# NVIDIA/OpenSeq2Seq

Hardware: AMD Instinct MI355X
Metric: audio-frames/sec/node Jasper10x5 bf16 (train step, objects = input feature frames) (higher is better)
Workload: dtype bf16; 1 GPU; Jasper 10x5 DR (jasper10x5_LibriSpeech_nvgrad_masks) full train step: log-mel front end from int16 PCM resident in HBM+fwd+bwd+NovoGrad/LARC/Backoff, B=32/GPU, durations U[2,16.7]s padded to the batch max, F=64, V=29; global_batch=32, parallelism=dp1, skipped_steps=0

## Files before the change

openseq2seq_amd/csrc/conv1d_wgrad.hip:

```cpp
#include <stdlib.h>

#include <cstdlib>
#include "os2s_common.hpp"
#include "os2s_split_reduce.hpp"
#include <mutex>

namespace os2s {

struct WgradArgs {
  const bf16_t* x;
  const bf16_t* dy;
  float* dw;
  const int32_t* in_len;
  int B, Tin, Tout, Cin, Cout, K, stride, dil, padL;
  int NCO, NCI, NTP, NSPLIT, steps_per_split, use_atomic;
  float* part;
  int xrows, xrows_pad;
  int xbuf_bytes, steptab_bytes;
  long long x_ld;
  int accumulate;
  float* ws_slabs;
  int* ws_cnt;
  int ws_nslabs, ncu, force_split;
  int xcd_order;
  int NG;
  const bf16_t* gx[8];
  const bf16_t* gdy[8];
  float* gdw[8];
  unsigned long long* dbg;
  int dbg_mode;
};

__device__ __forceinline__ int wgrad_xcd_rank(int b, int n) {
  const int q = n >> 3, r = n & 7, x = b & 7;
  return (x < r ? x * (q + 1) : r * (q + 1) + (x - r) * q) + (b >> 3);
}

__device__ __forceinline__ void dma16w(const void* gsrc, char* lds_wave_base) {
  __builtin_amdgcn_global_load_lds(
      (const __attribute__((address_space(1))) void*)gsrc,
      (__attribute__((address_space(3))) void*)lds_wave_base, 16, 0, 0);
}

__device__ __forceinline__ bf16x4 lds_tr(const char* p) {
  return __builtin_amdgcn_ds_read_tr16_b64_v4bf16(
      (__attribute__((address_space(3))) bf16x4*)p);
}

template <int TAPS, int COT>
__device__ __forceinline__ void wgrad_lockstep_unit(const WgradArgs& p, const int unit, const int tp, char* smem) {
  constexpr int BT = 64;
  constexpr int NW = COT / 32, NTHR = NW * 64, NSUB = COT / 128;
  const int tid = threadIdx.x, lane = tid & 63;
  const int wid = __builtin_amdgcn_readfirstlane(tid >> 6);
  const int wm = wid >> 1, wn = wid & 1;
  const int ysub = wm >> 1, wmi = wm & 1;
  const int split = unit / (p.NCO * p.NCI);
  const int rem = unit - split * (p.NCO * p.NCI);
  const int co0 = (rem / p.NCI) * COT, ci0 = (rem % p.NCI) * 128;
  const int k0 = tp * TAPS;
  const int ntaps = min(TAPS, p.K - k0);

  const int ybuf_bytes = NSUB * BT * 256;
  const int xbuf_bytes = p.xrows_pad * 256;
  char* const ybuf0 = smem;
  char* const xbuf0 = smem + 2 * ybuf_bytes;
  const char* const zero = reinterpret_cast<const char*>(g_zero_page);

  const int tchunks = (p.Tout + BT - 1) / BT;
  auto nlive = [&](int b) -> int {
    if (!p.in_len) return tchunks;
    const int l = min(max(p.in_len[b], 0), p.Tin);
    if (l <= 0) return 0;
    return min(tchunks, (l + p.padL + BT * p.stride - 1) / (BT * p.stride));
  };
  int total_live = 0;
  for (int b = 0; b < p.B; ++b) total_live += nlive(b);
  const int sps = (total_live + p.NSPLIT - 1) / p.NSPLIT;
  const int s_begin = split * sps;
  const int s_end = min(total_live, s_begin + sps);
  const int nsteps = max(0, s_end - s_begin);
  int cur_b = 0, cur_c = 0;
  {
    int acc_steps = 0;
    while (cur_b < p.B && acc_steps + nlive(cur_b) <= s_begin) { acc_steps += nlive(cur_b); ++cur_b; }
    cur_c = s_begin - acc_steps;
  }

  auto stage = [&](int step, int buf) {
    const int b = min(cur_b, p.B - 1);
    const int t0 = cur_c * BT;
    ++cur_c;
    if (cur_c >= nlive(b)) {
      cur_c = 0;
      ++cur_b;
      while (cur_b < p.B && nlive(cur_b) == 0) ++cur_b;
    }
    int len_b = p.Tin;
    if (p.in_len) {
      int l = p.in_len[b];
      len_b = l < 0 ? 0 : (l < p.Tin ? l : p.Tin);
    }
    char* yd = ybuf0 + buf * ybuf_bytes;
    const bf16_t* dyb = p.dy + (long long)b * p.Tout * p.Cout;
#pragma unroll
    for (int it = 0; it < (NSUB * 16) / NW; ++it) {
      const int base = (it * NW + wid) * 64;
      const int q = base + lane;
      const int sub = q >> 10, row = (q & 1023) >> 4, ps = q & 15;
      const int u = (ps >> 1) ^ ((row & 3) << 1);
      const int ch = co0 + sub * 128 + ((u << 1) | (ps & 1)) * 8;
      const int t = t0 + row;
      const bool ok = (t < p.Tout) && (ch < p.Cout);
      const void* src = ok ? (const void*)(dyb + (long long)t * p.Cout + ch)
                           : (const void*)(zero + ps * 16);
      dma16w(src, yd + base * 16);
    }
    char* xd = xbuf0 + buf * xbuf_bytes;
    const bf16_t* xb = p.x + (long long)b * p.Tin * p.x_ld;
    const int tin0 = t0 * p.stride + k0 * p.dil - p.padL;
    const int npieces = p.xrows_pad * 16;
    for (int base = wid * 64; base < npieces; base += NTHR) {
      const int q = base + lane;
      const int row = q >> 4, ps = q & 15;
      const int u = (ps >> 1) ^ ((row & 3) << 1);
      const int ch = ci0 + ((u << 1) | (ps & 1)) * 8;
      const int tin = tin0 + row;
      const bool ok = (row < p.xrows) && (tin >= 0) && (tin < len_b) && (ch < p.Cin);
      const void* src = ok ? (const void*)(xb + (long long)tin * p.x_ld + ch)
                           : (const void*)(zero + ps * 16);
      dma16w(src, xd + base * 16);
    }
  };

  f32x16 acc[TAPS][2][2];
#pragma unroll
  for (int a = 0; a < TAPS; ++a)
#pragma unroll
    for (int i = 0; i < 2; ++i)
#pragma unroll
      for (int j = 0; j < 2; ++j)
#pragma unroll
        for (int e = 0; e < 16; ++e) acc[a][i][j][e] = 0.f;

  const int g16 = (lane >> 4) & 1;
  const int i16 = lane & 15;
  const int rsub = i16 >> 2;
  const int csub = (i16 & 3) * 8;
  const int lhi = lane >> 5;

  if (nsteps > 0) stage(0, 0);
  for (int step = 0; step < nsteps; ++step) {
    asm volatile("s_waitcnt vmcnt(0)" ::: "memory");
    __syncthreads();
    if (step + 1 < nsteps) stage(step + 1, (step + 1) & 1);
    const char* const ys = ybuf0 + (step & 1) * ybuf_bytes + ysub * (BT * 256);
    const char* const xs = xbuf0 + (step & 1) * xbuf_bytes;
    struct Frags { bf16x8 af[2]; bf16x8 bfr[TAPS][2]; };
    auto load_frags = [&](int kk) {
      Frags f;
#pragma unroll
      for (int i = 0; i < 2; ++i) {
        const int u = ((wmi * 64 + i * 32) >> 4) + g16;
        const int r0 = kk * 16 + lhi * 8 + rsub;
        const int r1 = r0 + 4;
        const bf16x4 lo = lds_tr(ys + r0 * 256 + ((u ^ ((r0 & 3) << 1)) << 5) + csub);
        const bf16x4 hi = lds_tr(ys + r1 * 256 + ((u ^ ((r1 & 3) << 1)) << 5) + csub);
        f.af[i] = __builtin_shufflevector(lo, hi, 0, 1, 2, 3, 4, 5, 6, 7);
      }
#pragma unroll
      for (int a = 0; a < TAPS; ++a)
#pragma unroll
        for (int j = 0; j < 2; ++j) {
          const int u = ((wn * 64 + j * 32) >> 4) + g16;
          const int r0 = (kk * 16 + lhi * 8 + rsub) * p.stride + a * p.dil;
          const int r1 = r0 + 4 * p.stride;
// ... 562 lines not shown
      const int row = qq >> 4, ps = qq & 15;
      const int u = (ps >> 1) ^ ((row & 3) << 1);
      const int ch = ci0 + (idx >> 4) * 128 + ((u << 1) | (ps & 1)) * 8;
      xv[it] = ch < p.Cin ? (row * (int)p.x_ld + ch) * 2 : (int)0x80000000;
    }
  }
  const unsigned long long dy_base = (unsigned long long)p.dy, x_base = (unsigned long long)p.x;
  const int ycol_bytes = __builtin_amdgcn_readfirstlane(p.Cout * 2);
  const int xcol_bytes = __builtin_amdgcn_readfirstlane((int)p.x_ld * 2);
  auto entry = [&](int i, int& b, int& t0, int& len_b) {
    const unsigned long long m = __ballot(scan <= i);
    int bb = __builtin_popcountll(m);
    bb = bb < p.B ? bb : p.B - 1;
    b = __builtin_amdgcn_readfirstlane(bb);
    const int before = b > 0 ? __builtin_amdgcn_readlane(scan, b - 1) : 0;
    t0 = (i - before) * BT;
    len_b = __builtin_amdgcn_readlane(len_l, b);
  };
  auto stage_y = [&](int b, int t0, int len_b, int slot) {
    int rows = len_b - t0;
    rows = rows < 0 ? 0 : (rows > BT ? BT : rows);
    rows = __builtin_amdgcn_readfirstlane(rows);
    const unsigned long long base =
        dy_base + ((unsigned long long)(unsigned)b * (unsigned)p.Tout + (unsigned)t0) * (unsigned)ycol_bytes;
    const __amdgpu_buffer_rsrc_t rs = __builtin_amdgcn_make_buffer_rsrc((void*)base, 0, rows * ycol_bytes, 0x00020000);
    char* const dst = smem + slot * TILE + grp * HALF;
#pragma unroll
    for (int it = 0; it < 4; ++it)
      __builtin_amdgcn_raw_ptr_buffer_load_lds(
          rs, (__attribute__((address_space(3))) void*)(dst + (it * 4 + wn) * 1024), 16, yv[it], 0, 0, 0);
  };
  auto stage_x = [&](int b, int t0, int len_b, int slot) {
    int rows = len_b - t0;
    rows = rows < 0 ? 0 : (rows > BT ? BT : rows);
    rows = __builtin_amdgcn_readfirstlane(rows);
    const unsigned long long base =
        x_base + ((unsigned long long)(unsigned)b * (unsigned)p.Tin + (unsigned)t0) * (unsigned)xcol_bytes;
    const __amdgpu_buffer_rsrc_t rs = __builtin_amdgcn_make_buffer_rsrc((void*)base, 0, rows * xcol_bytes, 0x00020000);
    char* const dst = smem + 3 * TILE + slot * TILE;
#pragma unroll
    for (int it = 0; it < 4; ++it)
      __builtin_amdgcn_raw_ptr_buffer_load_lds(
          rs, (__attribute__((address_space(3))) void*)(dst + (it * 8 + wid) * 1024), 16, xv[it], 0, 0, 0);
  };

  f32x16 acc[2][2][2];
#pragma unroll
  for (int e = 0; e < 2; ++e)
#pragma unroll
    for (int i = 0; i < 2; ++i)
#pragma unroll
      for (int j = 0; j < 2; ++j)
#pragma unroll
        for (int v = 0; v < 16; ++v) acc[e][i][j][v] = 0.f;

  const int lhi = lane >> 5;
  if (nsteps > 0) {
    const int g16 = (lane >> 4) & 1, i16 = lane & 15;
    const int rsub = i16 >> 2, csub = (i16 & 3) * 8;
    int ya[2][2], xa[2];
#pragma unroll
    for (int e = 0; e < 2; ++e)
#pragma unroll
      for (int i = 0; i < 2; ++i) {
        const int u = 4 * e + 2 * i + g16;
        ya[e][i] = grp * HALF + (lhi * 8 + rsub) * 256 + ((u ^ ((rsub & 3) << 1)) << 5) + csub;
      }
#pragma unroll
    for (int j = 0; j < 2; ++j) {
      const int u = 4 * (wn & 1) + 2 * j + g16;
      xa[j] = (wn >> 1) * HALF + (lhi * 8 + rsub) * 256 + ((u ^ ((rsub & 3) << 1)) << 5) + csub;
    }
    {
      int b, t0, len_b;
      entry(s_begin, b, t0, len_b);
      stage_y(b, t0, len_b, 0);
      stage_x(b, t0, len_b, 0);
      if (nsteps > 1) {
        entry(s_begin + 1, b, t0, len_b);
        stage_y(b, t0, len_b, 1);
        stage_x(b, t0, len_b, 1);
        asm volatile("s_waitcnt vmcnt(8)" ::: "memory");
      } else {
        asm volatile("s_waitcnt vmcnt(0)" ::: "memory");
      }
    }
    wpp_barrier();
    if (grp) wpp_barrier();

    const unsigned lds0 = (unsigned)(size_t)(__attribute__((address_space(3))) void*)smem;
    int yi = 0;
    for (int s = 0; s < nsteps; ++s) {
      const unsigned ys = lds0 + yi * TILE;
      const unsigned xs = lds0 + 3 * TILE + (s & 1) * TILE;
      const bool more = s + 2 < nsteps;
      bf16x8 xf[2][4], yf[2][4];
#pragma unroll
      for (int j = 0; j < 2; ++j) {
        xf[j][0] = lds_frag<0>(xs + xa[j]); xf[j][1] = lds_frag<1>(xs + xa[j]);
        xf[j][2] = lds_frag<2>(xs + xa[j]); xf[j][3] = lds_frag<3>(xs + xa[j]);
      }
#pragma unroll
      for (int i = 0; i < 2; ++i) {
        yf[i][0] = lds_frag<0>(ys + ya[0][i]); yf[i][1] = lds_frag<1>(ys + ya[0][i]);
        yf[i][2] = lds_frag<2>(ys + ya[0][i]); yf[i][3] = lds_frag<3>(ys + ya[0][i]);
      }
      int b2 = 0, t2 = 0, l2 = 0;
      if (more) {
        entry(s_begin + s + 2, b2, t2, l2);
        int y2 = yi + 2;
        y2 = y2 >= 3 ? y2 - 3 : y2;
        stage_y(b2, t2, l2, y2);
      }
      asm volatile("s_waitcnt lgkmcnt(0)" ::: "memory");
      wpp_barrier();
#pragma unroll
      for (int kk = 0; kk < 4; ++kk)
#pragma unroll
        for (int i = 0; i < 2; ++i)
#pragma unroll
          for (int j = 0; j < 2; ++j)
            acc[0][i][j] = __builtin_amdgcn_mfma_f32_32x32x16_bf16(yf[i][kk], xf[j][kk], acc[0][i][j], 0, 0, 0);
      wpp_barrier();
#pragma unroll
      for (int i = 0; i < 2; ++i) {
        yf[i][0] = lds_frag<0>(ys + ya[1][i]); yf[i][1] = lds_frag<1>(ys + ya[1][i]);
        yf[i][2] = lds_frag<2>(ys + ya[1][i]); yf[i][3] = lds_frag<3>(ys + ya[1][i]);
      }
      if (more) {
        asm volatile("s_waitcnt vmcnt(4)" ::: "memory");
        stage_x(b2, t2, l2, s & 1);
      } else {
        asm volatile("s_waitcnt vmcnt(0)" ::: "memory");
      }
      yi = yi + 1 >= 3 ? 0 : yi + 1;
      asm volatile("s_waitcnt lgkmcnt(0)" ::: "memory");
      wpp_barrier();
#pragma unroll
      for (int kk = 0; kk < 4; ++kk)
#pragma unroll
        for (int i = 0; i < 2; ++i)
#pragma unroll
          for (int j = 0; j < 2; ++j)
            acc[1][i][j] = __builtin_amdgcn_mfma_f32_32x32x16_bf16(yf[i][kk], xf[j][kk], acc[1][i][j], 0, 0, 0);
      wpp_barrier();
    }
    if (!grp) wpp_barrier();
  }
  __syncthreads();

  if (npiece > 1) {
    const int sidx = rank - nfull;
    auto at = [&](int v) -> f32x16& { return acc[v >> 2][(v >> 1) & 1][v & 1]; };
    if (!split_publish_and_reduce(at, p.ws_slabs + (size_t)sidx * f * kSplitSlabFloats,
                                  p.ws_cnt + sidx, piece, f, smem, tid))
      return;
  }

  const int l31 = lane & 31;
  const bool inside = __builtin_amdgcn_readfirstlane((co0 + 256 <= p.Cout && ci0 + 256 <= p.Cin) ? 1 : 0);
#pragma unroll
  for (int e = 0; e < 2; ++e) {
    const int cob = co0 + grp * 128 + e * 64, cib = ci0 + wn * 64;
    if (inside) {
      float* const base = p.dw + (long long)(cob + 4 * lhi) * p.Cin + cib + l31;
      float old[2][2][16];
      if (p.accumulate) {
#pragma unroll
        for (int i = 0; i < 2; ++i)
#pragma unroll
          for (int j = 0; j < 2; ++j)
#pragma unroll
            for (int v = 0; v < 16; ++v)
              old[i][j][v] = base[(long long)(i * 32 + (v & 3) + 8 * (v >> 2)) * p.Cin + j * 32];
#pragma unroll
        for (int i = 0; i < 2; ++i)
#pragma unroll
          for (int j = 0; j < 2; ++j)
#pragma unroll
            for (int v = 0; v < 16; ++v) acc[e][i][j][v] += old[i][j][v];
      }
#pragma unroll
      for (int i = 0; i < 2; ++i)
#pragma unroll
        for (int j = 0; j < 2; ++j)
#pragma unroll
          for (int v = 0; v < 16; ++v)
            base[(long long)(i * 32 + (v & 3) + 8 * (v >> 2)) * p.Cin + j * 32] = acc[e][i][j][v];
    } else {
#pragma unroll
      for (int i = 0; i < 2; ++i)
#pragma unroll
        for (int j = 0; j < 2; ++j) {
          const int ci = cib + j * 32 + l31;
#pragma unroll
          for (int v = 0; v < 16; ++v) {
            const int co = cob + i * 32 + (v & 3) + 8 * (v >> 2) + 4 * lhi;
            if (co < p.Cout && ci < p.Cin) {
              float* dst = p.dw + (long long)co * p.Cin + ci;
              float val = acc[e][i][j][v];
              if (p.accumulate) val += *dst;
              *dst = val;
            }
          }
        }
    }
  }
}

}

static int conv1d_wgrad_impl(os2s_stream_t stream, const uint16_t* x, long long x_row_stride,
                             const uint16_t* dy, float* dw, const int32_t* in_len, int B,
                             int Tin, int Cin, int Cout, int K, int stride, int dil,
                             int padL, int Tout, int accumulate, void* workspace,
                             size_t workspace_bytes);

static int wgrad_pp_min_units() {
  static const int v = [] { const char* e = getenv("OS2S_WGRAD_PP_MIN_UNITS"); return e ? atoi(e) : 8; }();
  return v;
}
static bool wgrad1x1_pp_auto(int B, int T, int Cin, int Cout, bool have_ws) {
  static const int mode = [] { const char* e = getenv("OS2S_WGRAD1X1_PP"); return e ? atoi(e) : -1; }();
  if (mode == 0) return false;
  if (mode == 1) return true;
  const long long rows = (long long)B * T;
  const int units = os2s::ceil_div(Cout, 256) * os2s::ceil_div(Cin, 256);
  return have_ws && rows >= 2048 && units >= 32;
}
static int g_wgrad_variant = -1;
static int g_wgrad_split = -1;
static int g_wgrad_sw_ablate = 0;
static int g_wgrad_xcd = 1;
static unsigned long long* g_wgrad_dbg = nullptr;
static int g_wgrad_dbg_mode = 0;
static os2s::OptionReg r_wg_variant("conv1d_wgrad.variant", [](double v) { g_wgrad_variant = (int)v; });
static os2s::OptionReg r_wg_split("conv1d_wgrad.split", [](double v) { g_wgrad_split = (int)v; });
static os2s::OptionReg r_wg_abl("conv1d_wgrad.sw_ablate", [](double v) { g_wgrad_sw_ablate = (int)v; });
static os2s::OptionReg r_wg_xcd("conv1d_wgrad.xcd_order", [](double v) { g_wgrad_xcd = v != 0 ? 1 : 0; });
static os2s::StampReg r_wg_stamps("conv1d_wgrad", [](void* stamps, int mode) {
  g_wgrad_dbg = (unsigned long long*)stamps;
  g_wgrad_dbg_mode = mode;
});

extern "C" int os2s_conv1d_wgrad_ws(os2s_stream_t stream, const uint16_t* x, long long x_row_stride,
                                    const uint16_t* dy, float* dw, const int32_t* in_len, int B,
                                    int Tin, int Cin, int Cout, int K, int stride, int dil,
                                    int padL, int Tout, int accumulate, void* workspace,
                                    size_t workspace_bytes) {
  return conv1d_wgrad_impl(stream, x, x_row_stride, dy, dw, in_len, B, Tin, Cin, Cout, K, stride,
                           dil, padL, Tout, accumulate, workspace, workspace_bytes);
}

extern "C" int os2s_conv1d_wgrad_ex(os2s_stream_t stream, const uint16_t* x, long long x_row_stride,
                                    const uint16_t* dy, float* dw, const int32_t* in_len, int B,
                                    int Tin, int Cin, int Cout, int K, int stride, int dil,
                                    int padL, int Tout, int accumulate) {
  return conv1d_wgrad_impl(stream, x, x_row_stride, dy, dw, in_len, B, Tin, Cin, Cout, K, stride,
                           dil, padL, Tout, accumulate, nullptr, 0);
}

extern "C" int os2s_conv1d_wgrad(os2s_stream_t stream, const uint16_t* x,
                                 const uint16_t* dy, float* dw,
                                 const int32_t* in_len, int B, int Tin, int Cin,
                                 int Cout, int K, int stride, int dil, int padL,
                                 int Tout, int accumulate) {
  return conv1d_wgrad_impl(stream, x, Cin, dy, dw, in_len, B, Tin, Cin, Cout, K, stride, dil,
                           padL, Tout, accumulate, nullptr, 0);
}

static int conv1d_wgrad_impl_g(os2s_stream_t stream, const uint16_t* x, long long x_row_stride,
                               const uint16_t* dy, float* dw, const int32_t* in_len, int B,
                               int Tin, int Cin, int Cout, int K, int stride, int dil,
                               int padL, int Tout, int accumulate, void* workspace,
                               size_t workspace_bytes, const os2s_cwgrad_group_t* groups, int ngroups);

static int conv1d_wgrad_impl(os2s_stream_t stream, const uint16_t* x, long long x_row_stride,
                             const uint16_t* dy, float* dw, const int32_t* in_len, int B,
                             int Tin, int Cin, int Cout, int K, int stride, int dil,
                             int padL, int Tout, int accumulate, void* workspace,
                             size_t workspace_bytes) {
  return conv1d_wgrad_impl_g(stream, x, x_row_stride, dy, dw, in_len, B, Tin, Cin, Cout, K, stride, dil, padL, Tout,
                             accumulate, workspace, workspace_bytes, nullptr, 1);
}

extern "C" int os2s_conv1d_wgrad_grouped_ws(os2s_stream_t stream, const os2s_cwgrad_group_t* groups, int ngroups,
                                            const int32_t* in_len, int B, int Tin, int Cin, int Cout, int K,
                                            int stride, int dil, int padL, int Tout, int accumulate,
                                            void* workspace, size_t workspace_bytes) {
  OS2S_REQUIRE(groups && ngroups >= 1 && ngroups <= 8);
  for (int i = 0; i < ngroups; ++i) OS2S_REQUIRE(groups[i].x && groups[i].dy && groups[i].dw);
  for (int i = 1; i < ngroups; ++i) OS2S_REQUIRE(groups[i].x_row_stride == groups[0].x_row_stride);
  int rc = OS2S_ERR_UNSUPPORTED;
  if (ngroups > 1)
    rc = conv1d_wgrad_impl_g(stream, groups[0].x, groups[0].x_row_stride, groups[0].dy, groups[0].dw, in_len, B, Tin,
                             Cin, Cout, K, stride, dil, padL, Tout, accumulate, workspace, workspace_bytes, groups,
                             ngroups);
  if (rc != OS2S_ERR_UNSUPPORTED) return rc;
  for (int i = 0; i < ngroups; ++i) {
    rc = conv1d_wgrad_impl(stream, groups[i].x, groups[i].x_row_stride, groups[i].dy, groups[i].dw, in_len, B, Tin,
                           Cin, Cout, K, stride, dil, padL, Tout, accumulate, workspace, workspace_bytes);
    if (rc != OS2S_OK) return rc;
  }
  return OS2S_OK;
}

static int conv1d_wgrad_impl_g(os2s_stream_t stream, const uint16_t* x, long long x_row_stride,
                               const uint16_t* dy, float* dw, const int32_t* in_len, int B,
                               int Tin, int Cin, int Cout, int K, int stride, int dil,
                               int padL, int Tout, int accumulate, void* workspace,
                               size_t workspace_bytes, const os2s_cwgrad_group_t* groups, int ngroups) {
  using namespace os2s;
  OS2S_REQUIRE(x_row_stride >= Cin && x_row_stride % 8 == 0);
  OS2S_REQUIRE(x && dy && dw);
  OS2S_REQUIRE(B >= 0 && Tin >= 1 && Tout >= 1 && Cin >= 8 && Cout >= 8 && K >= 1);
  OS2S_REQUIRE(Cin % 8 == 0 && Cout % 8 == 0 && stride >= 1 && dil >= 1);
  if (B == 0) return OS2S_OK;
  WgradArgs a;
  a.x = x; a.dy = dy; a.dw = dw; a.in_len = in_len;
  a.B = B; a.Tin = Tin; a.Tout = Tout; a.Cin = Cin; a.Cout = Cout; a.K = K;
  a.stride = stride; a.dil = dil; a.padL = padL; a.x_ld = x_row_stride;
  a.accumulate = accumulate ? 1 : 0;
  a.part = nullptr; a.ws_slabs = nullptr; a.ws_cnt = nullptr; a.ws_nslabs = 0; a.ncu = 256; a.force_split = g_wgrad_split;
  a.dbg = g_wgrad_dbg; a.dbg_mode = g_wgrad_dbg_mode; a.xcd_order = g_wgrad_xcd; a.NG = 1;
  for (int i = 0; i < 8; ++i) { a.gx[i] = nullptr; a.gdy[i] = nullptr; a.gdw[i] = nullptr; }
  if (groups) {
    a.NG = ngroups;
    for (int i = 0; i < ngroups; ++i) { a.gx[i] = groups[i].x; a.gdy[i] = groups[i].dy; a.gdw[i] = groups[i].dw; }
  }

  const bool pp_shape = stride == 1 && K >= 2 && B <= 64 && Cout >= 128 && Cin >= 64 &&
                        Tin < 65536 && Tout <= 255 * 64 && 63 + 3 * dil + 1 <= 96 &&
                        (long long)Tin * x_row_stride * 2 < (1ll << 30) &&
                        (long long)Tin * x_row_stride * 2 < (1ll << 31) &&
                        (long long)Tout * Cout * 2 < (1ll << 31);
  const int pp_units = ceil_div(Cout, 128) * ceil_div(Cin, 128) * ceil_div(K, kWppTaps);
  const bool sw_shape = pp_shape && 63 + 3 * dil + 1 <= kSwXInstr * 16 &&
                        Cout % 128 == 0 && Cin % 128 == 0;
  if (sw_shape && g_wgrad_variant == 3 && !groups) {
    a.NCO = ceil_div(Cout, 128);
    a.NCI = ceil_div(Cin, 128);
    a.NTP = ceil_div(K, kWppTaps);
    a.NSPLIT = 1; a.steps_per_split = 0; a.use_atomic = 0;
    a.xrows = 63 + (kWppTaps - 1) * dil + 1;
    a.xrows_pad = ceil_div(a.xrows, 4) * 4;
    a.xbuf_bytes = kSwXBuf;
    a.steptab_bytes = ceil_div(B * ceil_div(Tout, 64) * 4, 16) * 16;
    const size_t smem = (size_t)kSwRing * (kSwYBuf + kSwXBuf) + a.steptab_bytes;
    if (smem <= 160 * 1024) {
      static std::once_flag once_sw;
      static hipError_t attr_rc = hipSuccess;
      static int ncu = 256;
      std::call_once(once_sw, [] {
        attr_rc = hipFuncSetAttribute((const void*)conv1d_wgrad_sw_kernel<0>,
                                      hipFuncAttributeMaxDynamicSharedMemorySize, 160 * 1024);
#ifdef OS2S_SW_ABLATE
        for (const void* k : {(const void*)conv1d_wgrad_sw_kernel<1>, (const void*)conv1d_wgrad_sw_kernel<2>,
                              (const void*)conv1d_wgrad_sw_kernel<4>, (const void*)conv1d_wgrad_sw_kernel<8>,
                              (const void*)conv1d_wgrad_sw_kernel<3>, (const void*)conv1d_wgrad_sw_kernel<5>})
          if (attr_rc == hipSuccess) attr_rc = hipFuncSetAttribute(k, hipFuncAttributeMaxDynamicSharedMemorySize, 160 * 1024);
#endif
        int dev = 0, n = 0;
        if (hipGetDevice(&dev) == hipSuccess &&
            hipDeviceGetAttribute(&n, hipDeviceAttributeMultiprocessorCount, dev) == hipSuccess && n > 0)
          ncu = n;
      });
      if (attr_rc != hipSuccess) return OS2S_ERR_LAUNCH;
      a.ncu = ncu;
      const size_t slab_bytes = (size_t)kSplitSlabFloats * 4;
      if (workspace && workspace_bytes >= kSplitTicketBytes + 2 * slab_bytes) {
        a.ws_cnt = reinterpret_cast<int*>(workspace);
        a.ws_slabs = reinterpret_cast<float*>(reinterpret_cast<char*>(workspace) + kSplitTicketBytes);
        size_t n = (workspace_bytes - kSplitTicketBytes) / slab_bytes;
        const size_t cap = (size_t)3 * ncu;
        a.ws_nslabs = (int)(n < cap ? n : cap);
      }
      const int U = a.NCO * a.NCI * a.NTP;
      const int r = U % ncu;
      const int pieces = a.ws_nslabs < 16 * r ? a.ws_nslabs : 16 * r;
#ifdef OS2S_SW_ABLATE
      switch (g_wgrad_sw_ablate) {
        case 1: OS2S_LAUNCH(conv1d_wgrad_sw_kernel<1>, dim3(U + pieces), dim3(256), smem, (hipStream_t)stream, a); return OS2S_OK;
        case 2: OS2S_LAUNCH(conv1d_wgrad_sw_kernel<2>, dim3(U + pieces), dim3(256), smem, (hipStream_t)stream, a); return OS2S_OK;
        case 3: OS2S_LAUNCH(conv1d_wgrad_sw_kernel<3>, dim3(U + pieces), dim3(256), smem, (hipStream_t)stream, a); return OS2S_OK;
        case 4: OS2S_LAUNCH(conv1d_wgrad_sw_kernel<4>, dim3(U + pieces), dim3(256), smem, (hipStream_t)stream, a); return OS2S_OK;
        case 5: OS2S_LAUNCH(conv1d_wgrad_sw_kernel<5>, dim3(U + pieces), dim3(256), smem, (hipStream_t)stream, a); return OS2S_OK;
        case 8: OS2S_LAUNCH(conv1d_wgrad_sw_kernel<8>, dim3(U + pieces), dim3(256), smem, (hipStream_t)stream, a); return OS2S_OK;
        default: break;
      }
#endif
      OS2S_LAUNCH(conv1d_wgrad_sw_kernel<0>, dim3(U + pieces), dim3(256), smem, (hipStream_t)stream, a);
      return OS2S_OK;
    }
  }

  if (pp_shape && g_wgrad_variant != 0 && (groups || g_wgrad_variant == 1 || pp_units >= wgrad_pp_min_units())) {
    a.NCO = ceil_div(Cout, 128);
    a.NCI = ceil_div(Cin, 128);
    a.NTP = ceil_div(K, kWppTaps);
    a.NSPLIT = 1; a.steps_per_split = 0; a.use_atomic = 0;
    a.xrows = 63 + (kWppTaps - 1) * dil + 1;
    a.xrows_pad = ceil_div(a.xrows, 4) * 4;
    a.xbuf_bytes = 24 * 1024;
    a.steptab_bytes = ceil_div(B * ceil_div(Tout, 64) * 4, 16) * 16;
    const size_t smem = (size_t)2 * 64 * 256 + (size_t)3 * a.xbuf_bytes + a.steptab_bytes + (a.dbg ? 2 * 48 * 10 * 8 : 0);
    if (smem <= 160 * 1024) {
      static std::once_flag once;
      static hipError_t attr_rc = hipSuccess;
      static int ncu = 256;
      std::call_once(once, [] {
        attr_rc = hipFuncSetAttribute((const void*)conv1d_wgrad_pp_kernel<false>,
                                      hipFuncAttributeMaxDynamicSharedMemorySize, 160 * 1024);
        if (attr_rc == hipSuccess)
          attr_rc = hipFuncSetAttribute((const void*)conv1d_wgrad_pp_kernel<true>,
                                        hipFuncAttributeMaxDynamicSharedMemorySize, 160 * 1024);
        int dev = 0, n = 0;
        if (hipGetDevice(&dev) == hipSuccess &&
            hipDeviceGetAttribute(&n, hipDeviceAttributeMultiprocessorCount, dev) == hipSuccess && n > 0)
          ncu = n;
      });
      if (attr_rc != hipSuccess) return OS2S_ERR_LAUNCH;
      a.ncu = ncu;
      const size_t slab_bytes = (size_t)kSplitSlabFloats * 4;
      if (workspace && workspace_bytes >= kSplitTicketBytes + 2 * slab_bytes) {
        a.ws_cnt = reinterpret_cast<int*>(workspace);
        a.ws_slabs = reinterpret_cast<float*>(reinterpret_cast<char*>(workspace) + kSplitTicketBytes);
        size_t n = (workspace_bytes - kSplitTicketBytes) / slab_bytes;
        const size_t cap = (size_t)3 * ncu;
        a.ws_nslabs = (int)(n < cap ? n : cap);
      }
      const int U = a.NG * a.NCO * a.NCI * a.NTP;
      const int r = U % ncu;
      int pieces = a.ws_nslabs < 16 * r ? a.ws_nslabs : 16 * r;
      const int grid = U + pieces;
      if (a.dbg) {
        OS2S_LAUNCH(conv1d_wgrad_pp_kernel<true>, dim3(grid), dim3(512), smem, (hipStream_t)stream, a);
      } else {
        OS2S_LAUNCH(conv1d_wgrad_pp_kernel<false>, dim3(grid), dim3(512), smem, (hipStream_t)stream, a);
      }
      return OS2S_OK;
    }
  }

  if (groups) return OS2S_ERR_UNSUPPORTED;

  const bool pp1_shape = K == 1 && stride == 1 && padL == 0 && Tin == Tout && B <= 64 &&
                         Cout >= 128 && Cin >= 128 && x_row_stride * 2 * 64 < (1ll << 30) &&
                         (long long)Cout * 2 * 64 < (1ll << 30);
  if (pp1_shape && g_wgrad_variant != 0 && g_wgrad_variant != 1 &&
      (g_wgrad_variant == 2 || wgrad1x1_pp_auto(B, Tout, Cin, Cout, workspace != nullptr))) {
    a.NCO = ceil_div(Cout, 256);
    a.NCI = ceil_div(Cin, 256);
    a.NTP = 1;
    a.NSPLIT = 1; a.steps_per_split = 0; a.use_atomic = 0;
    a.xrows = 64; a.xrows_pad = 64; a.xbuf_bytes = 0; a.steptab_bytes = 0;
    static std::once_flag once1;
    static hipError_t attr_rc1 = hipSuccess;
    static int ncu1 = 256;
    std::call_once(once1, [] {
      attr_rc1 = hipFuncSetAttribute((const void*)conv1d_wgrad1x1_pp_kernel,
                                     hipFuncAttributeMaxDynamicSharedMemorySize, 160 * 1024);
      int dev = 0, n = 0;
      if (hipGetDevice(&dev) == hipSuccess &&
          hipDeviceGetAttribute(&n, hipDeviceAttributeMultiprocessorCount, dev) == hipSuccess && n > 0)
        ncu1 = n;
    });
    if (attr_rc1 != hipSuccess) return OS2S_ERR_LAUNCH;
    a.ncu = ncu1;
    const size_t slab_bytes = (size_t)kSplitSlabFloats * 4;
    if (workspace && workspace_bytes >= kSplitTicketBytes + 2 * slab_bytes) {
      a.ws_cnt = reinterpret_cast<int*>(workspace);
      a.ws_slabs = reinterpret_cast<float*>(reinterpret_cast<char*>(workspace) + kSplitTicketBytes);
      size_t n = (workspace_bytes - kSplitTicketBytes) / slab_bytes;
      const size_t cap = (size_t)3 * ncu1;
      a.ws_nslabs = (int)(n < cap ? n : cap);
    }
    const int U = a.NCO * a.NCI;
    const int r = U % ncu1;
    const int pieces = a.ws_nslabs < 16 * r ? a.ws_nslabs : 16 * r;
    WgradGroupTable none;
    none.ngroups = 0; none.total_units = 0;
    OS2S_LAUNCH(conv1d_wgrad1x1_pp_kernel, dim3(U + pieces), dim3(512), (size_t)160 * 1024,
                (hipStream_t)stream, a, none);
    return OS2S_OK;
  }

  const int TAPS = K == 1 ? 1 : 2;
  const bool wide = (Cout % 256 == 0) && (K >= 8) && (Cout >= 512);
  const int COT = wide ? 256 : 128;
  a.NCO = ceil_div(Cout, COT);
  a.NCI = ceil_div(Cin, 128);
  a.NTP = ceil_div(K, TAPS);
  const int base_blocks = a.NCO * a.NCI * a.NTP;
  const int total_steps = B * ceil_div(Tout, 64);
  int nsplit = 1;
  if (accumulate) {
    const int target = wide ? 256 : 512;
    nsplit = ceil_div(target, base_blocks);
    const int max_split = total_steps / 8 > 0 ? total_steps / 8 : 1;
    if (nsplit > max_split) nsplit = max_split;
    if (nsplit < 1) nsplit = 1;
    if (os2s_deterministic()) nsplit = 1;
  }
  const long long dw_elems = (long long)K * Cout * Cin;
  if (workspace) {
    const long long part_room = workspace_bytes > kSplitTicketBytes
                                    ? (long long)((workspace_bytes - kSplitTicketBytes) / ((size_t)dw_elems * 4)) : 0;
    if (nsplit > part_room) nsplit = (int)part_room;
    if (nsplit < 1) nsplit = 1;
  }
  a.steps_per_split = ceil_div(total_steps, nsplit);
  a.NSPLIT = ceil_div(total_steps, a.steps_per_split);
  if (workspace && a.NSPLIT > 1)
    a.part = reinterpret_cast<float*>(reinterpret_cast<char*>(workspace) + kSplitTicketBytes);
  a.use_atomic = (accumulate && !a.part) ? 1 : 0;
  a.xrows = 63 * stride + (TAPS - 1) * dil + 1;
  a.xrows_pad = ceil_div(a.xrows, 4) * 4;
  const size_t smem = (size_t)2 * 64 * 2 * COT + (size_t)2 * a.xrows_pad * 256;
  if (smem > 160 * 1024) return OS2S_ERR_UNSUPPORTED;
  static std::once_flag once2;
  static hipError_t attr_rc2 = hipSuccess;
  std::call_once(once2, [] {
    if (hipFuncSetAttribute((const void*)conv1d_wgrad_kernel<2, 128>,
                            hipFuncAttributeMaxDynamicSharedMemorySize, 160 * 1024) != hipSuccess ||
        hipFuncSetAttribute((const void*)conv1d_wgrad_kernel<2, 256>,
                            hipFuncAttributeMaxDynamicSharedMemorySize, 160 * 1024) != hipSuccess ||
        hipFuncSetAttribute((const void*)conv1d_wgrad_kernel<1, 128>,
                            hipFuncAttributeMaxDynamicSharedMemorySize, 160 * 1024) != hipSuccess ||
        hipFuncSetAttribute((const void*)conv1d_wgrad_kernel<1, 256>,
                            hipFuncAttributeMaxDynamicSharedMemorySize, 160 * 1024) != hipSuccess)
      attr_rc2 = hipErrorUnknown;
  });
  if (attr_rc2 != hipSuccess) return OS2S_ERR_LAUNCH;
  const int nunits = a.NCO * a.NCI * a.NSPLIT;
  const int grid = ceil_div(nunits, 8) * 8 * a.NTP;
  if (wide) {
    if (TAPS == 1)
      OS2S_LAUNCH((conv1d_wgrad_kernel<1, 256>), dim3(grid), dim3(512), smem, (hipStream_t)stream, a);
    else
      OS2S_LAUNCH((conv1d_wgrad_kernel<2, 256>), dim3(grid), dim3(512), smem, (hipStream_t)stream, a);
  } else {
    if (TAPS == 1)
      OS2S_LAUNCH((conv1d_wgrad_kernel<1, 128>), dim3(grid), dim3(256), smem, (hipStream_t)stream, a);
    else
      OS2S_LAUNCH((conv1d_wgrad_kernel<2, 128>), dim3(grid), dim3(256), smem, (hipStream_t)stream, a);
  }
  if (a.part) {
    const int blocks = ceil_div(dw_elems, 256) < 2048 ? ceil_div(dw_elems, 256) : 2048;
    OS2S_LAUNCH(wgrad_split_sum_kernel, dim3(blocks), dim3(256), 0, (hipStream_t)stream,
                (const float*)a.part, dw, dw_elems, a.NSPLIT);
  }
  return OS2S_OK;
}


extern "C" int os2s_conv1x1_wgrad_grouped(os2s_stream_t stream, const os2s_wgrad_group_t* groups, int ngroups,
                                          const int32_t* in_len, int B, int T) {
  using namespace os2s;
  OS2S_REQUIRE(groups && ngroups >= 1 && ngroups <= kMaxWgradGroups && B >= 0 && T >= 1);
  if (B == 0) return OS2S_OK;
  WgradGroupTable gt;
  gt.ngroups = ngroups;
  int tiles = 0;
  for (int i = 0; i < ngroups; ++i) {
    const os2s_wgrad_group_t& s = groups[i];
    OS2S_REQUIRE(s.x && s.dy && s.dw && s.Cin >= 8 && s.Cout >= 8 && s.Cin % 8 == 0 && s.Cout % 8 == 0);
    OS2S_REQUIRE(s.x_row_stride >= s.Cin && s.x_row_stride % 8 == 0);
    tiles += ceil_div(s.Cout, 128) * ceil_div(s.Cin, 128);
  }
  const int total_steps = B * ceil_div(T, 64);
  int nsplit = ceil_div(512, tiles);
  const int max_split = total_steps / 8 > 0 ? total_steps / 8 : 1;
  if (nsplit > max_split) nsplit = max_split;
  if (tiles >= 256 || nsplit < 1 || os2s_deterministic()) nsplit = 1;
  WgradArgs a;
  a.x = nullptr; a.dy = nullptr; a.dw = nullptr; a.in_len = in_len;
  a.B = B; a.Tin = T; a.Tout = T; a.Cin = 0; a.Cout = 0; a.K = 1;
  a.stride = 1; a.dil = 1; a.padL = 0; a.x_ld = 0; a.accumulate = 1;
  a.part = nullptr; a.ws_slabs = nullptr; a.ws_cnt = nullptr; a.ws_nslabs = 0; a.ncu = 256; a.force_split = -1;
  a.dbg = nullptr; a.dbg_mode = 0; a.xcd_order = g_wgrad_xcd; a.NG = 1;
  a.NCO = 0; a.NCI = 0; a.NTP = 1;
  a.steps_per_split = ceil_div(total_steps, nsplit);
  a.NSPLIT = ceil_div(total_steps, a.steps_per_split);
  a.use_atomic = 1;
  a.xrows = 64; a.xrows_pad = 64; a.xbuf_bytes = 0; a.steptab_bytes = 0;
  int units = 0;
  for (int i = 0; i < kMaxWgradGroups; ++i) {
    const os2s_wgrad_group_t& s = groups[i < ngroups ? i : 0];
    WgradGroup& g = gt.g[i];
    g.x = s.x; g.dy = s.dy; g.dw = s.dw; g.x_ld = s.x_row_stride;
    g.Cin = s.Cin; g.Cout = s.Cout; g.NCI = ceil_div(s.Cin, 128);
    g.unit_begin = units;
    if (i < ngroups) units += ceil_div(s.Cout, 128) * g.NCI * a.NSPLIT;
  }
  gt.total_units = units;
  const size_t smem = (size_t)2 * 64 * 2 * 128 + (size_t)2 * a.xrows_pad * 256;
  static std::once_flag once;
  static hipError_t attr_rc = hipSuccess;
  std::call_once(once, [] {
    attr_rc = hipFuncSetAttribute((const void*)conv1d_wgrad_grouped_kernel,
                                  hipFuncAttributeMaxDynamicSharedMemorySize, 160 * 1024);
  });
  if (attr_rc != hipSuccess) return OS2S_ERR_LAUNCH;
  OS2S_LAUNCH(conv1d_wgrad_grouped_kernel, dim3(units), dim3(256), smem, (hipStream_t)stream, a, gt);
  return OS2S_OK;
}


extern "C" int os2s_conv1x1_wgrad_grouped_ws(os2s_stream_t stream, const os2s_wgrad_group_t* groups, int ngroups,
                                             const int32_t* in_len, int B, int T, void* workspace,
                                             size_t workspace_bytes) {
  using namespace os2s;
  OS2S_REQUIRE(groups && ngroups >= 1 && ngroups <= kMaxWgradGroups && B >= 0 && T >= 1);
  if (B == 0) return OS2S_OK;
  bool pp = B <= 64 && (long long)B * T >= 2048 && workspace != nullptr;
  for (int i = 0; i < ngroups && pp; ++i) {
    const os2s_wgrad_group_t& s = groups[i];
    OS2S_REQUIRE(s.x && s.dy && s.dw && s.Cin >= 8 && s.Cout >= 8 && s.Cin % 8 == 0 && s.Cout % 8 == 0);
    OS2S_REQUIRE(s.x_row_stride >= s.Cin && s.x_row_stride % 8 == 0);
    pp = s.Cin >= 128 && s.Cout >= 128 && s.x_row_stride * 2 * 64 < (1ll << 30) &&
         (long long)s.Cout * 2 * 64 < (1ll << 30);
  }
  if (!pp) return os2s_conv1x1_wgrad_grouped(stream, groups, ngroups, in_len, B, T);
  WgradGroupTable gt;
  gt.ngroups = ngroups;
  int units = 0;
  for (int i = 0; i < kMaxWgradGroups; ++i) {
    const os2s_wgrad_group_t& s = groups[i < ngroups ? i : 0];
    WgradGroup& g = gt.g[i];
    g.x = s.x; g.dy = s.dy; g.dw = s.dw; g.x_ld = s.x_row_stride;
    g.Cin = s.Cin; g.Cout = s.Cout; g.NCI = ceil_div(s.Cin, 256);
    g.unit_begin = units;
    if (i < ngroups) units += ceil_div(s.Cout, 256) * g.NCI;
  }
  gt.total_units = units;
  WgradArgs a;
  a.x = gt.g[0].x; a.dy = gt.g[0].dy; a.dw = gt.g[0].dw; a.in_len = in_len;
  a.B = B; a.Tin = T; a.Tout = T; a.Cin = gt.g[0].Cin; a.Cout = gt.g[0].Cout; a.K = 1;
  a.stride = 1; a.dil = 1; a.padL = 0; a.x_ld = gt.g[0].x_ld;
  a.accumulate = 1;
  a.part = nullptr; a.ws_slabs = nullptr; a.ws_cnt = nullptr; a.ws_nslabs = 0; a.ncu = 256; a.force_split = g_wgrad_split;
  a.dbg = nullptr; a.dbg_mode = 0; a.xcd_order = g_wgrad_xcd; a.NG = 1;
  a.NCO = units; a.NCI = 1; a.NTP = 1;
  a.NSPLIT = 1; a.steps_per_split = 0; a.use_atomic = 0;
  a.xrows = 64; a.xrows_pad = 64; a.xbuf_bytes = 0; a.steptab_bytes = 0;
  static std::once_flag once;
  static hipError_t attr_rc = hipSuccess;
  static int ncu = 256;
  std::call_once(once, [] {
    attr_rc = hipFuncSetAttribute((const void*)conv1d_wgrad1x1_pp_kernel,
                                  hipFuncAttributeMaxDynamicSharedMemorySize, 160 * 1024);
    int dev = 0, n = 0;
    if (hipGetDevice(&dev) == hipSuccess &&
        hipDeviceGetAttribute(&n, hipDeviceAttributeMultiprocessorCount, dev) == hipSuccess && n > 0)
      ncu = n;
  });
  if (attr_rc != hipSuccess) return OS2S_ERR_LAUNCH;
  a.ncu = ncu;
  const size_t slab_bytes = (size_t)kSplitSlabFloats * 4;
  if (workspace_bytes >= kSplitTicketBytes + 2 * slab_bytes) {
    a.ws_cnt = reinterpret_cast<int*>(workspace);
    a.ws_slabs = reinterpret_cast<float*>(reinterpret_cast<char*>(workspace) + kSplitTicketBytes);
    size_t n = (workspace_bytes - kSplitTicketBytes) / slab_bytes;
    const size_t cap = (size_t)3 * ncu;
    a.ws_nslabs = (int)(n < cap ? n : cap);
  }
  const int r = units % ncu;
  const int pieces = a.ws_nslabs < 16 * r ? a.ws_nslabs : 16 * r;
  OS2S_LAUNCH(conv1d_wgrad1x1_pp_kernel, dim3(units + pieces), dim3(512), (size_t)160 * 1024,
              (hipStream_t)stream, a, gt);
  return OS2S_OK;
}

extern "C" int os2s_gemm_wgrad_grouped(os2s_stream_t stream, const os2s_wgrad_group_t* groups, int ngroups,
                                       long long M, int accumulate, void* workspace, size_t workspace_bytes) {
  using namespace os2s;
  OS2S_REQUIRE(groups && ngroups >= 1 && ngroups <= kMaxWgradGroups && M >= 1 && M < (1ll << 30));
  WgradGroupTable gt;
  gt.ngroups = ngroups;
  int units = 0;
  for (int i = 0; i < kMaxWgradGroups; ++i) {
    const os2s_wgrad_group_t& s = groups[i < ngroups ? i : 0];
    OS2S_REQUIRE(s.x && s.dy && s.dw && s.Cin >= 128 && s.Cout >= 128 && s.Cin % 8 == 0 && s.Cout % 8 == 0);
    OS2S_REQUIRE(s.x_row_stride >= s.Cin && s.x_row_stride % 8 == 0);
    OS2S_REQUIRE(s.x_row_stride * 2 * 64 < (1ll << 30) && (long long)s.Cout * 2 * 64 < (1ll << 30));
    WgradGroup& g = gt.g[i];
    g.x = s.x; g.dy = s.dy; g.dw = s.dw; g.x_ld = s.x_row_stride;
    g.Cin = s.Cin; g.Cout = s.Cout; g.NCI = ceil_div(s.Cin, 256);
    g.unit_begin = units;
    if (i < ngroups) units += ceil_div(s.Cout, 256) * g.NCI;
  }
  gt.total_units = units;
  WgradArgs a;
  a.x = gt.g[0].x; a.dy = gt.g[0].dy; a.dw = gt.g[0].dw; a.in_len = nullptr;
  a.B = 1; a.Tin = (int)M; a.Tout = (int)M; a.Cin = gt.g[0].Cin; a.Cout = gt.g[0].Cout; a.K = 1;
  a.stride = 1; a.dil = 1; a.padL = 0; a.x_ld = gt.g[0].x_ld;
  a.accumulate = accumulate ? 1 : 0;
  a.part = nullptr; a.ws_slabs = nullptr; a.ws_cnt = nullptr; a.ws_nslabs = 0; a.ncu = 256; a.force_split = g_wgrad_split;
  a.dbg = nullptr; a.dbg_mode = 0; a.xcd_order = g_wgrad_xcd; a.NG = 1;
  a.NCO = units; a.NCI = 1; a.NTP = 1;
  a.NSPLIT = 1; a.steps_per_split = 0; a.use_atomic = 0;
  a.xrows = 64; a.xrows_pad = 64; a.xbuf_bytes = 0; a.steptab_bytes = 0;
  static std::once_flag once;
  static hipError_t attr_rc = hipSuccess;
  static int ncu = 256;
  std::call_once(once, [] {
    attr_rc = hipFuncSetAttribute((const void*)conv1d_wgrad1x1_pp_kernel,
                                  hipFuncAttributeMaxDynamicSharedMemorySize, 160 * 1024);
    int dev = 0, n = 0;
    if (hipGetDevice(&dev) == hipSuccess &&
        hipDeviceGetAttribute(&n, hipDeviceAttributeMultiprocessorCount, dev) == hipSuccess && n > 0)
      ncu = n;
  });
  if (attr_rc != hipSuccess) return OS2S_ERR_LAUNCH;
  a.ncu = ncu;
  const size_t slab_bytes = (size_t)kSplitSlabFloats * 4;
  if (workspace && workspace_bytes >= kSplitTicketBytes + 2 * slab_bytes) {
    a.ws_cnt = reinterpret_cast<int*>(workspace);
    a.ws_slabs = reinterpret_cast<float*>(reinterpret_cast<char*>(workspace) + kSplitTicketBytes);
    size_t n = (workspace_bytes - kSplitTicketBytes) / slab_bytes;
    const size_t cap = (size_t)3 * ncu;
    a.ws_nslabs = (int)(n < cap ? n : cap);
  }
  const int r = units % ncu;
  const int pieces = a.ws_nslabs < 16 * r ? a.ws_nslabs : 16 * r;
  OS2S_LAUNCH(conv1d_wgrad1x1_pp_kernel, dim3(units + pieces), dim3(512), (size_t)160 * 1024,
              (hipStream_t)stream, a, gt);
  return OS2S_OK;
}
```

openseq2seq_amd/csrc/os2s_split_reduce.hpp:

```cpp
#pragma once
#include "os2s_common.hpp"

namespace os2s {

constexpr int kSplitSlabFloats = 256 * 256;
constexpr size_t kSplitTicketBytes = 4096;

template <int NT = 512, int NV = 8, class At>
__device__ __forceinline__ bool split_publish_and_reduce(At&& at, float* slab0, int* ticket,
                                                        int piece, int f, char* smem, int tid) {
  static_assert(NT * NV * 16 == kSplitSlabFloats, "a partial tile is 256 x 256 floats");
  float* const mine = slab0 + (size_t)piece * kSplitSlabFloats;
#pragma unroll
  for (int v = 0; v < NV; ++v)
#pragma unroll
    for (int g4 = 0; g4 < 4; ++g4) {
      const f32x16& a = at(v);
      f32x4 x = {a[4 * g4], a[4 * g4 + 1], a[4 * g4 + 2], a[4 * g4 + 3]};
      *reinterpret_cast<f32x4*>(mine + (((v * 4 + g4) * NT + tid) << 2)) = x;
    }
  asm volatile("s_waitcnt vmcnt(0)" ::: "memory");
  __syncthreads();
  if (tid == 0) {
    __builtin_amdgcn_fence(__ATOMIC_RELEASE, "agent");
    asm volatile("s_waitcnt vmcnt(0)" ::: "memory");
    const int old = __hip_atomic_fetch_add(ticket, 1, __ATOMIC_RELAXED, __HIP_MEMORY_SCOPE_AGENT);
    *reinterpret_cast<volatile int*>(smem) = old;
  }
  __syncthreads();
  const int old = *reinterpret_cast<volatile int*>(smem);
  if (old != f - 1) return false;
  if (tid == 0) {
    __builtin_amdgcn_fence(__ATOMIC_ACQUIRE, "agent");
    __hip_atomic_store(ticket, 0, __ATOMIC_RELAXED, __HIP_MEMORY_SCOPE_AGENT);
  }
  __syncthreads();
#pragma unroll
  for (int h = 0; h < NV / 2; ++h) {
    f32x4 sum[8];
#pragma unroll
    for (int v = 0; v < 8; ++v) sum[v] = f32x4{0.f, 0.f, 0.f, 0.f};
    for (int jj = 0; jj < f; ++jj) {
      const float* const sl = slab0 + (size_t)jj * kSplitSlabFloats;
      f32x4 t[8];
#pragma unroll
      for (int v = 0; v < 8; ++v)
        t[v] = *reinterpret_cast<const f32x4*>(sl + ((((h * 2 + (v >> 2)) * 4 + (v & 3)) * NT + tid) << 2));
#pragma unroll
      for (int v = 0; v < 8; ++v) sum[v] += t[v];
    }
#pragma unroll
    for (int v = 0; v < 8; ++v) {
      f32x16& a = at(h * 2 + (v >> 2));
#pragma unroll
      for (int e = 0; e < 4; ++e) a[4 * (v & 3) + e] = sum[v][e];
    }
  }
  return true;
}

template <int NT, int NV, class At>
__device__ __forceinline__ bool split_publish(At&& at, float* slab0, int* ticket, int piece, int f, char* smem, int tid) {
  static_assert(NT * NV * 16 == kSplitSlabFloats, "a partial tile is 256 x 256 floats");
  float* const mine = slab0 + (size_t)piece * kSplitSlabFloats;
#pragma unroll
  for (int v = 0; v < NV; ++v)
#pragma unroll
    for (int g4 = 0; g4 < 4; ++g4) {
      const f32x16& a = at(v);
      f32x4 x = {a[4 * g4], a[4 * g4 + 1], a[4 * g4 + 2], a[4 * g4 + 3]};
      *reinterpret_cast<f32x4*>(mine + (((v * 4 + g4) * NT + tid) << 2)) = x;
    }
  asm volatile("s_waitcnt vmcnt(0)" ::: "memory");
  __syncthreads();
  if (tid == 0) {
    __builtin_amdgcn_fence(__ATOMIC_RELEASE, "agent");
    asm volatile("s_waitcnt vmcnt(0)" ::: "memory");
    const int old = __hip_atomic_fetch_add(ticket, 1, __ATOMIC_RELAXED, __HIP_MEMORY_SCOPE_AGENT);
    *reinterpret_cast<volatile int*>(smem) = old;
  }
  __syncthreads();
  const int old = *reinterpret_cast<volatile int*>(smem);
  if (old != f - 1) return false;
  if (tid == 0) {
    __builtin_amdgcn_fence(__ATOMIC_ACQUIRE, "agent");
    __hip_atomic_store(ticket, 0, __ATOMIC_RELAXED, __HIP_MEMORY_SCOPE_AGENT);
  }
  __syncthreads();
  return true;
}
template <int NT, int NV, class Emit>
__device__ __forceinline__ void split_reduce_emit(const float* slab0, int f, int tid, Emit&& emit8) {
#pragma unroll
  for (int h = 0; h < NV / 2; ++h) {
    f32x4 sum[8];
#pragma unroll
    for (int k = 0; k < 8; ++k) sum[k] = f32x4{0.f, 0.f, 0.f, 0.f};
    for (int jj = 0; jj < f; ++jj) {
      const float* const sl = slab0 + (size_t)jj * kSplitSlabFloats;
      f32x4 t[8];
#pragma unroll
      for (int k = 0; k < 8; ++k)
        t[k] = *reinterpret_cast<const f32x4*>(sl + (((h * 8 + k) * NT + tid) << 2));
#pragma unroll
      for (int k = 0; k < 8; ++k) sum[k] += t[k];
    }
    emit8(h, sum);
  }
}

__host__ __device__ __forceinline__ int split_factor(int r, int G, float round_us, int fmax, int max_pieces) {
  int f = 1;
  float best = round_us;
  for (int ff = 2; ff <= fmax; ++ff) {
    if (r * ff > max_pieces) break;
    const float t = (float)((r * ff + G - 1) / G) * round_us / ff + 20.f + 1.5f * ff + 0.17f * (r * ff);
    if (t < 0.95f * best) { best = t; f = ff; }
  }
  return f;
}

}
```

Baseline: 951,200 frames/sec.

## Use two-level tree reduction for split-K wgrad partial tiles

Replaces the single-ticket serial finish, where the last arriving piece sums all f partial slabs, with a two-level tree. Pieces are grouped in fours, and the last piece of each group sums its group into the group's first slab. The globally last group finisher then sums only the group results. This shortens the serial tail reduction on the critical path at the cost of extra atomics, an extra slab write pass, and a packed bit-field ticket counter.

```diff
diff --git a/openseq2seq_amd/csrc/conv1d_wgrad.hip b/openseq2seq_amd/csrc/conv1d_wgrad.hip
--- a/openseq2seq_amd/csrc/conv1d_wgrad.hip
+++ b/openseq2seq_amd/csrc/conv1d_wgrad.hip
@@ -22,6 +22,7 @@
   float* ws_slabs;
   int* ws_cnt;
   int ws_nslabs, ncu, force_split;
+  int serial_finish = 0;
   int xcd_order;
   int NG;
   const bf16_t* gx[8];
@@ -890,9 +891,10 @@
   if (npiece > 1) {
     const int sidx = rank - nfull;
     auto at = [&](int v) -> f32x16& { return acc[v >> 2][(v >> 1) & 1][v & 1]; };
-    if (!split_publish_and_reduce(at, p.ws_slabs + (size_t)sidx * f * kSplitSlabFloats,
-                                  p.ws_cnt + sidx, piece, f, smem, tid))
-      return;
+    float* const slabs = p.ws_slabs + (size_t)sidx * f * kSplitSlabFloats;
+    const bool last = split_publish_and_reduce_tree(at, slabs, p.ws_cnt + sidx, piece, f, p.serial_finish ? 16 : 4,
+                                                    smem, tid);
+    if (!last) return;
   }
 
   const int l31 = lane & 31;
@@ -968,12 +970,14 @@
 }
 static int g_wgrad_variant = -1;
 static int g_wgrad_split = -1;
+static int g_wgrad_split_finish = 1;
 static int g_wgrad_sw_ablate = 0;
 static int g_wgrad_xcd = 1;
 static unsigned long long* g_wgrad_dbg = nullptr;
 static int g_wgrad_dbg_mode = 0;
 static os2s::OptionReg r_wg_variant("conv1d_wgrad.variant", [](double v) { g_wgrad_variant = (int)v; });
 static os2s::OptionReg r_wg_split("conv1d_wgrad.split", [](double v) { g_wgrad_split = (int)v; });
+static os2s::OptionReg r_wg_finish("conv1d_wgrad.split_finish", [](double v) { g_wgrad_split_finish = v != 0 ? 1 : 0; });
 static os2s::OptionReg r_wg_abl("conv1d_wgrad.sw_ablate", [](double v) { g_wgrad_sw_ablate = (int)v; });
 static os2s::OptionReg r_wg_xcd("conv1d_wgrad.xcd_order", [](double v) { g_wgrad_xcd = v != 0 ? 1 : 0; });
 static os2s::StampReg r_wg_stamps("conv1d_wgrad", [](void* stamps, int mode) {
@@ -1218,6 +1222,7 @@
     const int pieces = a.ws_nslabs < 16 * r ? a.ws_nslabs : 16 * r;
     WgradGroupTable none;
     none.ngroups = 0; none.total_units = 0;
+    a.serial_finish = g_wgrad_split_finish ? 0 : 1;
     OS2S_LAUNCH(conv1d_wgrad1x1_pp_kernel, dim3(U + pieces), dim3(512), (size_t)160 * 1024,
                 (hipStream_t)stream, a, none);
     return OS2S_OK;
@@ -1405,6 +1410,7 @@
   }
   const int r = units % ncu;
   const int pieces = a.ws_nslabs < 16 * r ? a.ws_nslabs : 16 * r;
+  a.serial_finish = g_wgrad_split_finish ? 0 : 1;
   OS2S_LAUNCH(conv1d_wgrad1x1_pp_kernel, dim3(units + pieces), dim3(512), (size_t)160 * 1024,
               (hipStream_t)stream, a, gt);
   return OS2S_OK;
@@ -1462,6 +1468,7 @@
   }
   const int r = units % ncu;
   const int pieces = a.ws_nslabs < 16 * r ? a.ws_nslabs : 16 * r;
+  a.serial_finish = g_wgrad_split_finish ? 0 : 1;
   OS2S_LAUNCH(conv1d_wgrad1x1_pp_kernel, dim3(units + pieces), dim3(512), (size_t)160 * 1024,
               (hipStream_t)stream, a, gt);
   return OS2S_OK;
diff --git a/openseq2seq_amd/csrc/os2s_split_reduce.hpp b/openseq2seq_amd/csrc/os2s_split_reduce.hpp
--- a/openseq2seq_amd/csrc/os2s_split_reduce.hpp
+++ b/openseq2seq_amd/csrc/os2s_split_reduce.hpp
@@ -42,6 +42,94 @@
     for (int v = 0; v < 8; ++v) sum[v] = f32x4{0.f, 0.f, 0.f, 0.f};
     for (int jj = 0; jj < f; ++jj) {
       const float* const sl = slab0 + (size_t)jj * kSplitSlabFloats;
+      f32x4 t[8];
+#pragma unroll
+      for (int v = 0; v < 8; ++v)
+        t[v] = *reinterpret_cast<const f32x4*>(sl + ((((h * 2 + (v >> 2)) * 4 + (v & 3)) * NT + tid) << 2));
+#pragma unroll
+      for (int v = 0; v < 8; ++v) sum[v] += t[v];
+    }
+#pragma unroll
+    for (int v = 0; v < 8; ++v) {
+      f32x16& a = at(h * 2 + (v >> 2));
+#pragma unroll
+      for (int e = 0; e < 4; ++e) a[4 * (v & 3) + e] = sum[v][e];
+    }
+  }
+  return true;
+}
+
+template <int NT = 512, int NV = 8, class At>
+__device__ __forceinline__ bool split_publish_and_reduce_tree(At&& at, float* slab0, int* ticket,
+                                                             int piece, int f, int gs, char* smem, int tid) {
+  const int ng = (gs >= f || f > 4 * gs || gs > 4) ? 1 : (f + gs - 1) / gs;
+  const int grp = ng > 1 ? piece / gs : 0;
+  float* const mine = slab0 + (size_t)piece * kSplitSlabFloats;
+#pragma unroll
+  for (int v = 0; v < NV; ++v)
+#pragma unroll
+    for (int g4 = 0; g4 < 4; ++g4) {
+      const f32x16& a = at(v);
+      f32x4 x = {a[4 * g4], a[4 * g4 + 1], a[4 * g4 + 2], a[4 * g4 + 3]};
+      *reinterpret_cast<f32x4*>(mine + (((v * 4 + g4) * NT + tid) << 2)) = x;
+    }
+  asm volatile("s_waitcnt vmcnt(0)" ::: "memory");
+  __syncthreads();
+  if (ng > 1) {
+    const int gsize = f - grp * gs < gs ? f - grp * gs : gs;
+    if (tid == 0) {
+      __builtin_amdgcn_fence(__ATOMIC_RELEASE, "agent");
+      asm volatile("s_waitcnt vmcnt(0)" ::: "memory");
+      const int old = __hip_atomic_fetch_add(ticket, 1 << (4 * grp), __ATOMIC_RELAXED, __HIP_MEMORY_SCOPE_AGENT);
+      *reinterpret_cast<volatile int*>(smem) = (old >> (4 * grp)) & 15;
+    }
+    __syncthreads();
+    if (*reinterpret_cast<volatile int*>(smem) != gsize - 1) return false;
+    float* const gslab = slab0 + (size_t)grp * gs * kSplitSlabFloats;
+    if (gsize > 1) {
+      if (tid == 0) __builtin_amdgcn_fence(__ATOMIC_ACQUIRE, "agent");
+      __syncthreads();
+      for (int q = 0; q < NV * 4; q += 4) {
+        f32x4 sum[4];
+#pragma unroll
+        for (int k = 0; k < 4; ++k) sum[k] = f32x4{0.f, 0.f, 0.f, 0.f};
+        for (int jj = 0; jj < gsize; ++jj) {
+          const float* const sl = gslab + (size_t)jj * kSplitSlabFloats;
+          f32x4 t[4];
+#pragma unroll
+          for (int k = 0; k < 4; ++k) t[k] = *reinterpret_cast<const f32x4*>(sl + (((q + k) * NT + tid) << 2));
+#pragma unroll
+          for (int k = 0; k < 4; ++k) sum[k] += t[k];
+        }
+#pragma unroll
+        for (int k = 0; k < 4; ++k) *reinterpret_cast<f32x4*>(gslab + (((q + k) * NT + tid) << 2)) = sum[k];
+      }
+      asm volatile("s_waitcnt vmcnt(0)" ::: "memory");
+    }
+    __syncthreads();
+  }
+  if (tid == 0) {
+    __builtin_amdgcn_fence(__ATOMIC_RELEASE, "agent");
+    asm volatile("s_waitcnt vmcnt(0)" ::: "memory");
+    const int old = __hip_atomic_fetch_add(ticket, ng > 1 ? 1 << 16 : 1, __ATOMIC_RELAXED, __HIP_MEMORY_SCOPE_AGENT);
+    *reinterpret_cast<volatile int*>(smem) = ng > 1 ? old >> 16 : old;
+  }
+  __syncthreads();
+  if (*reinterpret_cast<volatile int*>(smem) != (ng > 1 ? ng : f) - 1) return false;
+  if (tid == 0) {
+    __builtin_amdgcn_fence(__ATOMIC_ACQUIRE, "agent");
+    __hip_atomic_store(ticket, 0, __ATOMIC_RELAXED, __HIP_MEMORY_SCOPE_AGENT);
+  }
+  __syncthreads();
+  const int n = ng > 1 ? ng : f;
+  const size_t stride = (size_t)(ng > 1 ? gs : 1) * kSplitSlabFloats;
+#pragma unroll
+  for (int h = 0; h < NV / 2; ++h) {
+    f32x4 sum[8];
+#pragma unroll
+    for (int v = 0; v < 8; ++v) sum[v] = f32x4{0.f, 0.f, 0.f, 0.f};
+    for (int jj = 0; jj < n; ++jj) {
+      const float* const sl = slab0 + (size_t)jj * stride;
       f32x4 t[8];
 #pragma unroll
       for (int v = 0; v < 8; ++v)
```

Result: no change. 950,600 frames/sec, median of 2 (-0.1%).
